# Research-Implementation/AudioVidSum-A-Multi-Modal-Approach-to-Video-Summarization

Hardware: AMD Instinct MI355X
Metric: frames/sec end-to-end (extract+fuse+score), 224x224 + 16kHz (higher is better)
Workload: dtype f16x2; 1 GPU; configs[1]: SumMe-shape batch, 25 videos x ~1800 frames (45143 frames/GPU), visual-only resnet50 extractor (batch-stat BN, the reference's 4-frame BatchNorm micro-batches inside each video) + AVBiLSTM attention scorer + mean-threshold selection; frames_per_gpu=45143, videos_per_gpu=25, extractor=resnet50, frames_per_group=4, chunk_frames=16384, parallelism=videos sharded x1, no data-path collective, selected_frames_rank0=22823

## Files before the change

### audiovidsum-a-multi-modal-approach-to-video-summarization_amd/_abi.py

```python
import ctypes
import os
from ctypes import POINTER, c_char_p, c_double, c_float, c_int, c_int64, c_size_t, c_uint, c_void_p

import torch

_PKG_DIR = os.path.dirname(os.path.abspath(__file__))
STUDY = os.environ.get("AVS_STUDY_LIB") == "1"
_FLAVOUR = os.environ.get("AVS_STUDY_LIB")
LIB_PATH = os.path.join(_PKG_DIR, "lib", "libavsum_hip_study.so" if STUDY else
                        "libavsum_hip_fp16emu.so" if _FLAVOUR == "fp16emu" else "libavsum_hip.so")
HEADER_PATH = os.path.join(os.path.dirname(_PKG_DIR), "include", "avsum_hip.h")

AVS_F32, AVS_BF16, AVS_F32_ACC64, AVS_F32_SPLIT, AVS_F16X2 = 0, 1, 2, 3, 4
AVS_W_ROWS, AVS_W_KSTEP32 = 0, 1
TILE_AUTO, TILE_128, TILE_256, TILE_224, STAGING_GENERIC = 0, 1, 2, 3, 4
CLUSTER_PACKED = 8
X_F16P8, Y_F16P8, RES_F16P8 = 1, 2, 4
LSTM_AUTO, LSTM_STREAM, LSTM_RESIDENT_20_8, LSTM_RESIDENT_16_8 = 0, 1, 2, 3
LSTM_SPLIT4 = 4
ACT_NONE, ACT_RELU = 0, 1
BIAS_NONE, BIAS_COL, BIAS_ROW = 0, 1, 2
E_UNSUPPORTED = -6


class AvsError(RuntimeError):
    pass


class ConvDesc(ctypes.Structure):
    _fields_ = [
        ("dtype", c_int),
        ("n", c_int), ("h", c_int), ("w", c_int),
        ("cin", c_int), ("kh", c_int), ("kw", c_int),
        ("sh", c_int), ("sw", c_int), ("ph", c_int), ("pw", c_int),
        ("ho", c_int), ("wo", c_int), ("cout", c_int),
        ("x_img_stride", c_int64), ("x_row_stride", c_int64), ("x_px_stride", c_int64),
        ("w_row_stride", c_int64), ("y_px_stride", c_int64),
        ("act", c_int), ("alpha", c_float), ("w_layout", c_int), ("variant", c_int), ("formats", c_int),
    ]


P = c_void_p
_SIGNATURES = {
    "avs_abi_version": (c_int, []),
    "avs_last_error": (c_char_p, []),
    "avs_device_info": (c_int, [c_int, POINTER(c_int), POINTER(c_int), POINTER(c_int64), c_char_p, c_int]),
    "avs_f16x2_pack_f32": (c_int, [P, P, c_int64, P]),
    "avs_f16x2_unpack_f32": (c_int, [P, P, c_int64, P]),
    "avs_f16p8_pack_f32": (c_int, [P, P, c_int64, P]),
# ... 158 lines not shown
```

### audiovidsum-a-multi-modal-approach-to-video-summarization_amd/cnn.py

```python
from typing import NamedTuple

import torch
import torch.nn as nn

from . import ops

RESNET_MEAN = (0.485, 0.456, 0.406)
RESNET_STD = (0.229, 0.224, 0.225)


class _NoTorchForward(nn.Module):
    def forward(self, *a, **k):
        raise RuntimeError("this module only holds parameters; the trunk runs through the HIP runner")


class Bottleneck(_NoTorchForward):
    expansion = 4

    def __init__(self, inplanes, planes, stride=1, downsample=None):
        super().__init__()
        self.conv1 = nn.Conv2d(inplanes, planes, 1, bias=False)
        self.bn1 = nn.BatchNorm2d(planes)
        self.conv2 = nn.Conv2d(planes, planes, 3, stride, 1, bias=False)
        self.bn2 = nn.BatchNorm2d(planes)
# ... 50 lines not shown
        self.kstep = ops.weights_kstep32(rows) if rows.shape[1] % step == 0 else None

    def conv_operand(self):
        return (self.kstep, 1) if self.kstep is not None else (self.rows, 0)


class Step(NamedTuple):
    name: str
    form: str
    inp: str = "finished"
    out: str = "finished"
    res: str = "none"
    block: int = -1
    geom: tuple = None
    cluster: int = 1
    packed: bool = False


class ResNet50Runner:

    def __init__(self, trunk, dtype=torch.float32, bn_mode="batch", f32_split=False):
        if bn_mode not in ("batch", "folded"):
            raise ValueError("bn_mode must be 'batch' (reference-faithful) or 'folded'")
        self.trunk, self.dtype, self.bn_mode = trunk, dtype, bn_mode
        self.h2 = f32_split == "f16x2" and dtype == torch.float32
        self.f32_split = bool(f32_split) and not self.h2 and dtype == torch.float32
        self.code = ops.dtype_code(dtype, "f16x2" if self.h2 else self.f32_split)
        self.ecode = self.code if self.h2 else ops.dtype_code(dtype)
        self.fuse_conv_bn = True
        self.fuse_min_rows, self.fuse_ratio_num, self.fuse_ratio_den = 128, 2, 1
        self.bn_local = True
        self.bn_cluster = True
        self.pack_groups = True
        self.fused_stem = True
        self.stem_raw = True
        self.defer_bn_apply = True
        self.defer_res_apply = True
        self.fold_input_bn = True
        self.gram_finish_min_k = 128
        self.p8_blocks = (0, 1, 3, 4, 5) if self.h2 else ()
        self._key = None
        self._w = None
        self._plans = {}

    block_hook = None

    def _blocks(self):
        for li in range(4):
            for b, blk in enumerate(self.trunk[4 + li]):
                yield f"layer{li + 1}.{b}", blk

    def _pair_ok(self):
        b0 = self.trunk[4][0]
        d = b0.downsample
        return d is not None and b0.conv1.weight[0].numel() == d[0].weight[0].numel() and b0.bn1.eps == d[1].eps

    def _prepare(self):
        key = tuple((p.data_ptr(), p._version) for p in self.trunk.parameters()) + (self.dtype,)
        if self._w is not None and key == self._key:
            return self._w
        t, dt = self.trunk, self.dtype
        pack = ops.f16x2_pack if self.h2 else (lambda r: r)

        def bn(m):
            return (m.weight.detach().float().contiguous(), m.bias.detach().float().contiguous(), float(m.eps),
                    m.running_mean.detach().float(), m.running_var.detach().float())
# ... 144 lines not shown
        return group_frames, gsz, bool((sizes == gsz).all())

    def _conv(self, st, w, x, x_aff, groups, residual=None, res_aff=None):
        (geom, xs, _), (wt, (gamma, beta, eps, rmean, rvar)) = st.geom, w[st.name]
        n, cin, kh, ho, wo, cout = geom[0], geom[3], geom[4], geom[10], geom[11], geom[12]
        dev, dt, stem = x.device, self.dtype, st.block < 0
        relu = not st.name.endswith("downsample")
        act = ops.ACT_RELU if relu else ops.ACT_NONE
        grows, gmax = groups[ho * wo]
        wsel, layout = wt.conv_operand()
        y = torch.empty((n, ho, wo, cout), dtype=dt, device=dev)

        def pooled():
            return torch.empty((n, (ho + 2 - 3) // 2 + 1, (wo + 2 - 3) // 2 + 1, cout), dtype=dt, device=dev)

        if st.form == "gram":
            x2d = x.view(-1, cin)
            if self.h2:
                sc, sf = ops.bn_gram_affine_h2(x2d, wt.rows, gmax, gamma, beta, eps, x_aff, store_input=x_aff is not None)
                if st.out == "p8":
                    y = ops.P8.empty((n, ho, wo, cout), dev)
                ops.conv2d_affine(self.code, n, geom[1], geom[2], cin, geom[6], geom[7], ho, wo, cout, x, *xs, wsel,
                                  wsel.stride(0), y, cout, gmax, sc, sf, residual, relu, res_aff, w_layout=layout)
            else:
                ops.conv1x1_gram_bn(x2d, wt.rows, gmax, gamma, beta, eps, y.view(-1, cout), residual, relu, x_aff, res_aff,
                                    finish_input=cin >= self.gram_finish_min_k)
            return y, None

        def conv(**kw):
            return ops.conv2d_raw(self.code, *geom, x, *xs, wsel, wsel.stride(0), y, cout, algo_k=147 if stem else None,
                                  algo_in_elems=x.numel() if stem else None, w_layout=layout, **kw)

        if st.form in ("local", "cluster"):
            conv(act=act, bnlocal=(gmax, gamma, beta, eps, residual), cluster=st.cluster, packed=st.packed)
            return (ops.pool2d(y, "max", 3, 2, 1, pooled(), code=self.ecode) if stem else y), None
        affine = None
        if st.form == "folded":
            conv()
            scale = (gamma / torch.sqrt(rvar + eps)).contiguous()
            affine, grows, gmax = (scale.view(1, -1), (beta - rmean * scale).contiguous().view(1, -1)), None, 0
        else:
            if x_aff is not None:
                if st.form == "stats" and kh == 3:
                    affine = conv(bnstats=(gmax, gamma, beta, eps), x_affine=(x_aff[0], x_aff[1], True))
                if affine is None:
                    xg = groups[geom[1] * geom[2]]
                    ops.bn_apply(x.view(-1, cin), x_aff[0], x_aff[1], xg[0], xg[1], None, ops.ACT_RELU, x.view(-1, cin),
                                 code=self.ecode)
            if st.form == "stats" and affine is None:
                affine = conv(bnstats=(gmax, gamma, beta, eps))
            elif st.form == "split":
                conv()
                affine = ops.bn_batch_stats(y.view(-1, cout), grows, gamma, beta, eps, code=self.ecode)
            if st.out == "deferred":
                return y, affine
        if stem:
            return ops.bn_maxpool(y, affine[0], affine[1], grows, relu, 3, 2, 1, pooled(), code=self.ecode), None
        ops.bn_apply(y.view(-1, cout), affine[0], affine[1], grows, gmax, residual, act, y.view(-1, cout), code=self.ecode)
        return y, None

    def _gram_pair(self, st, w, x, x_aff, gmax):
        wcat, gcat, bcat, eps, c1n = w[st.name]
        block = st.name.split(".conv1+")[0]
        geom, xs, _ = st.geom
        n, h, cin = geom[0], geom[1], geom[3]
        x2d = x.view(-1, cin)
        if self.h2:
# ... 398 lines not shown
```

### audiovidsum-a-multi-modal-approach-to-video-summarization_amd/csrc/igemm.hip

```cpp
#include "avs_internal.h"
#include "igemm_params.h"
#include <type_traits>

__device__ __attribute__((aligned(16))) unsigned int avs_zero16[4];

#ifdef AVS_STUDY
#define AVS_DEBUG_BIT(p, bit) ((p).debug & (bit))
#else
#define AVS_DEBUG_BIT(p, bit) 0
#endif

#define AVS_GLDS16(src, dst)                                                                        \
  __builtin_amdgcn_global_load_lds((const __attribute__((address_space(1))) void*)(src),            \
                                   (__attribute__((address_space(3))) void*)(dst), 16, 0, 0)

__device__ __forceinline__ void avs_split_bf16(const float4& p0, const float4& p1, bf16x8& hi, bf16x8& lo) {
  const float v[8] = {p0.x, p0.y, p0.z, p0.w, p1.x, p1.y, p1.z, p1.w};
  unsigned h[4], l[4];
#pragma unroll
  for (int j = 0; j < 4; ++j) {
    const unsigned short h0 = avs_f32_to_bf16(v[2 * j]), h1 = avs_f32_to_bf16(v[2 * j + 1]);
    const unsigned short l0 = avs_f32_to_bf16(v[2 * j] - avs_bf16_to_f32(h0));
    const unsigned short l1 = avs_f32_to_bf16(v[2 * j + 1] - avs_bf16_to_f32(h1));
    h[j] = (unsigned)h0 | ((unsigned)h1 << 16);
// ... 1561 lines not shown
                         (pl.tall || (long long)p.K * 4 <= g_rowb_threshold_bytes) &&
                         p.KW == 1 && p.K == p.cin && p.K % 32 == 0 && p.K >= 64 &&
                         p.sh == 1 && p.sw == 1 && p.ph == 0 && p.pw == 0 && p.x_row_stride == (long long)p.Wo * p.x_px_stride &&
                         p.x_img_stride == (long long)p.HoWo * p.x_px_stride && p.x_px_stride % 16 == 0 &&
                         256 * p.x_px_stride * 3 + (long long)p.K * 3 < (1ll << 31),
                     AVS_E_UNSUPPORTED,
                     "%s: an AVS_F16P8 input is taken by avs_conv2d_nhwc_bnstats for 1x1 / stride-1 convolutions on dense rows, "
                     "cin a multiple of 32 (>= 64), the input row stride a multiple of 16", who);
  }
  if (p.affine) {
    pl.tall = !(!narrow && (tile_mode == AVS_TILE_128 || (tile_mode == AVS_TILE_AUTO && p.K <= AVS_RULE_AFFINE_128_MAX_K)));
    if (!pl.tall && (long long)p.K * 4 > g_rowb_threshold_bytes) pl.tall = true;
  }
  pl.tile_rows = p.tile_rows ? p.tile_rows : (pl.tall ? 256 : 128);
  pl.tiles_m = ((long long)p.M + pl.tile_rows - 1) / pl.tile_rows;
  AVS_PLAN_REQUIRE(pl.tiles_m * pl.tiles_n < (1ll << 31), AVS_E_SHAPE, "%s: too many tiles", who);
  pl.grid = pl.tiles_m * pl.tiles_n;

  pl.spatial = !(p.ph == 0 && p.pw == 0 && (p.HoWo / p.Wo - 1) * p.sh + (p.K / (p.cin * p.KW)) - 1 < p.H &&
                 (p.Wo - 1) * p.sw + p.KW - 1 < p.W);
  pl.lin_stride = -1;
  if (!pl.spatial && p.KW == 1 && p.K == p.cin && p.sh == 1 && p.sw == 1) {
    if (p.HoWo == 1)
      pl.lin_stride = p.x_img_stride;
    else if (p.x_row_stride == (long long)p.Wo * p.x_px_stride && p.x_img_stride == (long long)p.HoWo * p.x_px_stride)
      pl.lin_stride = p.x_px_stride;
  }
  if (p.tile_rows && dtype == AVS_F16X2) {
    pl.local224 = igemm_h2_local224_ok(p, dtype, pl.lin_stride);
    AVS_PLAN_REQUIRE(pl.local224 || p.cluster <= 1, AVS_E_UNSUPPORTED, "%s: the clustered form runs on the 224-row tile only", who);
    AVS_PLAN_REQUIRE(pl.local224 || tile_mode != AVS_TILE_224, AVS_E_UNSUPPORTED,
                     "%s: AVS_TILE_224 takes AVS_F16X2, groups of 193..224 rows, cout in multiples of 128, cin in multiples of 16", who);
    if (pl.local224) return AVS_OK;
  }

  pl.epi = EPI_ANY;
  if (p.tile_rows)
    pl.epi = EPI_BNLOCAL;
  else if (p.affine)
    pl.epi = EPI_AFFINE;
  else if (p.bias_mode == AVS_BIAS_NONE && p.act == AVS_ACT_NONE && p.alpha == 1.0f)
    pl.epi = stats ? EPI_STATS : EPI_PLAIN;
  else if (brelu)
    pl.epi = EPI_BRELU;
  const bool fast64_only = !(p.variant & AVS_STAGING_GENERIC) && p.cin % (64 / es) == 0 && p.cin % (128 / es) != 0 && p.K / p.cin <= 32;
  const bool short_k = pl.tall || fast64_only || (long long)p.K * es <= g_rowb_threshold_bytes;
  pl.rowb = short_k ? 64 : 128;
  pl.pipe = pl.rowb == 64 && !pl.acc64 && g_pipe3 && p.K * es > 2 * pl.rowb;
  pl.wr = pl.pipe && pl.tall ? 4 : 2;
  pl.fastk = !pl.acc64 && igemm_fastk_ok(p, pl.lin_stride, es, pl.rowb / es, pl.bn);
  if (pl.spatial && pl.pipe && pl.wr == 4 && pl.fastk && (es == 2 || pl.split == 2)) {
    if (pl.epi == EPI_STATS || pl.epi == EPI_BNLOCAL)
      pl.tap9 = igemm_tap9_ok(p, es);
    else if (pl.epi == EPI_BRELU && pl.split == 2)
      pl.tap9 = igemm_taps_ok(p);
  }
  pl.xin = in_affine && pl.tap9 && pl.split == 2 && pl.epi == EPI_STATS;
  pl.ap8 = p.x_p8 && pl.split == 2 && pl.epi == EPI_STATS && !pl.spatial && pl.pipe && pl.fastk;
  return AVS_OK;
}
#undef AVS_PLAN_REQUIRE

#define AVS_LAUNCH_RET(K)                                     \
  do {                                                        \
    hipLaunchKernelGGL(K, grid, dim3(256), 0, stream, p);     \
    return true;                                              \
// ... 140 lines not shown
  return igemm_run(pl, p, stream, who);
}

static int conv_geometry(const avs_conv_desc* d, bool has_bias, IgemmParams& p, const char* who) {
  AVS_REQUIRE(d != nullptr, AVS_E_ARG, "%s: null descriptor", who);
  AVS_REQUIRE(d->n >= 0 && d->h > 0 && d->w > 0 && d->cin > 0 && d->kh > 0 && d->kw > 0 && d->sh > 0 && d->sw > 0 &&
                  d->ph >= 0 && d->pw >= 0 && d->ho > 0 && d->wo > 0 && d->cout > 0,
              AVS_E_SHAPE, "%s: non-positive extent", who);
  AVS_REQUIRE((d->ho - 1) * d->sh - d->ph + d->kh - 1 < d->h + d->ph &&
                  (d->wo - 1) * d->sw - d->pw + d->kw - 1 < d->w + d->pw,
              AVS_E_SHAPE, "%s: output extent %dx%d exceeds what input %dx%d allows", who, d->ho, d->wo, d->h, d->w);
  const long long rows = (long long)d->n * d->ho * d->wo;
  AVS_REQUIRE(rows < (1ll << 31), AVS_E_SHAPE, "%s: %lld output pixels exceed int32", who, rows);
  p.M = (int)rows;
  p.N = d->cout;
  p.K = d->kh * d->kw * d->cin;
  p.HoWo = d->ho * d->wo;
  p.Wo = d->wo;
  p.H = d->h;
  p.W = d->w;
  p.cin = d->cin;
  p.KW = d->kw;
  p.sh = d->sh;
  p.sw = d->sw;
  p.ph = d->ph;
  p.pw = d->pw;
  p.x_img_stride = d->x_img_stride;
  p.x_row_stride = d->x_row_stride;
  p.x_px_stride = d->x_px_stride;
  p.ldb = d->w_row_stride;
  AVS_REQUIRE(d->w_layout == AVS_W_ROWS || d->w_layout == AVS_W_KSTEP32, AVS_E_ARG, "%s: bad w_layout %d", who,
              d->w_layout);
  p.w_kstep = d->w_layout == AVS_W_KSTEP32 ? 1 : 0;
  AVS_REQUIRE((d->variant & ~15) == 0, AVS_E_ARG, "%s: bad variant %d", who, d->variant);
  p.variant = d->variant;
  AVS_REQUIRE((d->formats & ~(AVS_X_F16P8 | AVS_Y_F16P8 | AVS_RES_F16P8)) == 0, AVS_E_ARG, "%s: bad formats %d", who, d->formats);
  AVS_REQUIRE(d->formats == 0 || d->dtype == AVS_F16X2, AVS_E_UNSUPPORTED, "%s: AVS_F16P8 operands belong to the AVS_F16X2 forms", who);
  p.x_p8 = (d->formats & AVS_X_F16P8) ? 1 : 0;
  p.y_p8 = (d->formats & AVS_Y_F16P8) ? 1 : 0;
  p.res_p8 = (d->formats & AVS_RES_F16P8) ? 1 : 0;
  AVS_REQUIRE(!p.w_kstep || (d->dtype != AVS_F32_ACC64 && p.K % (d->dtype == AVS_BF16 ? 32 : 16) == 0), AVS_E_UNSUPPORTED,
              "%s: the reduction-step-major weight layout needs a reduction that is a multiple of a 64-byte step (K = %d)",
              who, p.K);
  p.ldc = d->y_px_stride;
  p.alpha = d->alpha;
  p.act = d->act;
  p.bias_mode = has_bias ? AVS_BIAS_COL : AVS_BIAS_NONE;
  AVS_REQUIRE(p.ldb >= p.K, AVS_E_SHAPE, "%s: w_row_stride %lld < kh*kw*cin=%d", who, p.ldb, p.K);
  return AVS_OK;
}

static void conv_operands(IgemmParams& p, const void* d_x, const void* d_w, const float* d_bias, void* d_y) {
  p.x = (const char*)d_x;
  p.w = (const char*)d_w;
  p.y = (char*)d_y;
  p.bias = d_bias;
}

extern "C" int avs_conv2d_nhwc(const avs_conv_desc* d, const void* d_x, const void* d_w, const float* d_bias,
                               void* d_y, avs_stream_t stream) {
  IgemmParams p{};
  int st = conv_geometry(d, d_bias != nullptr, p, "avs_conv2d_nhwc");
  if (st != AVS_OK) return st;
  conv_operands(p, d_x, d_w, d_bias, d_y);
  return igemm_launch(d->dtype, p, 1, (hipStream_t)stream, "avs_conv2d_nhwc");
}

// ... 132 lines not shown
  AVS_CHECK_LAUNCH(who);
  return AVS_OK;
}

extern "C" int avs_conv2d_nhwc_bnstats(const avs_conv_desc* d, const void* d_x, const void* d_w, void* d_y,
                                       int64_t rows_per_group, const float* d_gamma, const float* d_beta, float eps,
                                       float* d_scale, float* d_shift, void* d_ws, int64_t ws_bytes,
                                       avs_stream_t stream) {
  return conv_bnstats(d, d_x, d_w, d_y, rows_per_group, d_gamma, d_beta, eps, d_scale, d_shift, d_ws, ws_bytes, nullptr,
                      nullptr, 0, stream, "avs_conv2d_nhwc_bnstats");
}

extern "C" int avs_conv2d_nhwc_bnstats_xin(const avs_conv_desc* d, const void* d_x, const void* d_w, void* d_y,
                                           int64_t rows_per_group, const float* d_gamma, const float* d_beta, float eps,
                                           float* d_scale, float* d_shift, void* d_ws, int64_t ws_bytes,
                                           const float* d_in_scale, const float* d_in_shift, int in_relu,
                                           avs_stream_t stream) {
  const char* who = "avs_conv2d_nhwc_bnstats_xin";
  AVS_REQUIRE(d_in_scale && d_in_shift, AVS_E_ARG, "%s: in_scale / in_shift must be given", who);
  return conv_bnstats(d, d_x, d_w, d_y, rows_per_group, d_gamma, d_beta, eps, d_scale, d_shift, d_ws, ws_bytes, d_in_scale,
                      d_in_shift, in_relu, stream, who);
}


static int bnlocal_plan(const avs_conv_desc* d, int64_t rpg, IgemmParams& p, const char* who) {
  int st = conv_geometry(d, false, p, who);
  if (st != AVS_OK) return st;
  AVS_REQUIRE(rpg > 0, AVS_E_ARG, "%s: rows_per_group must be positive", who);
  if (p.M == 0) return AVS_OK;
  const int bn = p.N <= 64 ? 64 : 128;
  const long long per_tile = 256 / rpg;
  const bool h2 = d->dtype == AVS_F16X2;
  const int es = h2 ? 4 : 2;
  const bool ok = (g_bnlocal != 0) && (g_pipe3 != 0) && (d->dtype == AVS_BF16 || h2) && p.N % bn == 0 && p.M % rpg == 0 && rpg <= 256 &&
                  per_tile * rpg * 4 >= 256 * 3 && per_tile <= BNLOCAL_MAX_GROUPS && (long long)p.K * es > 128 &&
                  d->alpha == 1.0f && (p.ldc * es) % (h2 ? 32 : 16) == 0;
  AVS_REQUIRE(ok, AVS_E_UNSUPPORTED,
              "%s: needs bf16 / f16x2, cout a multiple of %d, equal groups of 43..256 rows that fill 3/4 of a 256-row "
              "tile, a reduction of more than 128 bytes, aligned output rows", who, bn);
  p.tiles_n = p.N / bn;
  p.tile_rows = (int)(per_tile * rpg);
  return AVS_OK;
}

static int bncluster_plan(const avs_conv_desc* d, int64_t rpg, int cluster, IgemmParams& p, const char* who) {
  int st = conv_geometry(d, false, p, who);
  if (st != AVS_OK) return st;
  AVS_REQUIRE(rpg > 0 && cluster >= 2 && cluster <= 16, AVS_E_ARG, "%s: rows_per_group > 0 and 2 <= cluster <= 16", who);
  if (p.M == 0) return AVS_OK;
  const bool ok = (g_bnlocal != 0) && (g_pipe3 != 0) && d->dtype == AVS_F16X2 && rpg % cluster == 0 && p.M % rpg == 0 &&
                  rpg / cluster > 192 && rpg / cluster <= 224 && p.N % 128 == 0 && (long long)p.K * 4 > 128 &&
                  d->alpha == 1.0f && (p.ldc * 4) % 32 == 0 && (d->variant & AVS_STAGING_GENERIC) == 0;
  AVS_REQUIRE(ok, AVS_E_UNSUPPORTED,
              "%s: needs AVS_F16X2, equal groups of `cluster` tiles of 193..224 rows each, cout a multiple of 128, a "
              "reduction of more than 128 bytes, aligned output rows", who);
  p.tiles_n = p.N / 128;
  p.tile_rows = (int)(rpg / cluster);
  p.rows_per_group = (int)rpg;
  p.cluster = cluster;
  if (d->variant & AVS_CLUSTER_PACKED) {
    const int64_t per_group = (rpg + 223) / 224;
    AVS_REQUIRE(rpg >= 224 && (rpg % 224 == 0 || rpg % 224 == 112) && per_group <= 16, AVS_E_UNSUPPORTED,
                "%s: AVS_CLUSTER_PACKED needs groups of a multiple of 112 rows, at least 224, that touch at most 16 tiles", who);
    p.tile_rows = 224;
    p.packed = (int)(rpg % 224 ? rpg / 112 : rpg / 224);
  }
  return AVS_OK;
}

static int64_t bncluster_workspace(const IgemmParams& p) {
  if (p.packed) return 64 + (int64_t)((p.M + 223) / 224) * p.tiles_n * 4 * 2 * 64 * 8;
  return 64 + (int64_t)(p.M / p.tile_rows) * p.tiles_n * 4 * 64 * 8;
// ... 149 lines not shown
```

### audiovidsum-a-multi-modal-approach-to-video-summarization_amd/csrc/local224.hip

```cpp
#include "avs_internal.h"
#include "igemm_params.h"
#include <type_traits>
#include <utility>

namespace {
constexpr int L_ROWS = 224;
constexpr int L_MT = L_ROWS / 32;
constexpr int L_BN = 128;
constexpr int L_CPRR = 4;
constexpr int L_STEP = 16;
constexpr int L_BUF = (L_ROWS + L_BN) * L_CPRR;
constexpr int L_P = 32 + 8;
constexpr unsigned L_OOB = 0x80000000u;

template <int OFF>
__device__ __forceinline__ uint4 lds_read_b128_at(unsigned byte_addr) {
  uint4 v;
  asm volatile("ds_read_b128 %0, %1 offset:%2" : "=v"(v) : "v"(byte_addr), "n"(OFF));
  return v;
}
template <int... I>
__device__ __forceinline__ void read_blocks(uint4 (&f)[L_MT], unsigned addr, std::integer_sequence<int, I...>) {
  ((f[I] = lds_read_b128_at<I * 32 * 64>(addr)), ...);
}
}

template <bool SPATIAL>
__global__ __launch_bounds__(256, 2) void igemm_h2_local224_kernel(IgemmParams p) {
  __shared__ uint4 lds[3 * L_BUF];

  const unsigned nwg = gridDim.x, orig = blockIdx.x;
  const unsigned q = nwg >> 3, rr = nwg & 7, xcd = orig & 7;
  const unsigned wg = (xcd < rr ? xcd * (q + 1) : rr * (q + 1) + (xcd - rr) * q) + (orig >> 3);
  int tn = wg % p.tiles_n;
  int tm = wg / p.tiles_n;
  if (p.packed) {
    const unsigned u_t = (unsigned)p.packed, tnn = (unsigned)p.tiles_n;
    const unsigned tiles_m = nwg / tnn;
    const unsigned full = (56u % u_t == 0u) ? (tiles_m / 56u) * 56u : 0u;
    if (orig < full * tnn) {
      const unsigned su = orig / (56u * tnn), l = orig - su * (56u * tnn);
      tn = (int)(l / 56u);
      tm = (int)(su * 56u + l % 56u);
    } else {
      const unsigned o2 = orig - full * tnn, unit = u_t * tnn;
      const unsigned u = o2 / unit, l = o2 - u * unit;
      const unsigned left = tiles_m - full - u * u_t, ul = left < u_t ? left : u_t;
      tn = (int)(l / ul);
      tm = (int)(full + u * u_t + l % ul);
    }
  } else if (p.cluster > 1) {
    const unsigned c = (unsigned)p.cluster, tnn = (unsigned)p.tiles_n;
    const unsigned tiles_m = nwg / tnn;
    const unsigned full = (8u % c == 0u) ? (tiles_m / 8u) * 8u : 0u;
    if (orig < full * tnn) {
      const unsigned su = orig / (8u * tnn), l = orig - su * (8u * tnn);
      tn = (int)(l >> 3);
      tm = (int)(su * 8u + (l & 7u));
    } else {
      const unsigned o2 = orig - full * tnn, unit = c * tnn;
      const unsigned u = o2 / unit, l = o2 - u * unit;
      tn = (int)(l / c);
      tm = (int)(full + u * c + l % c);
    }
  }
  const int m0 = tm * p.tile_rows;
  const int n0 = tn * L_BN;
  const int used = m0 + p.tile_rows <= p.M ? p.tile_rows : p.M - m0;

  const char* __restrict__ x = p.x;
  const char* __restrict__ w = p.w;
  char* __restrict__ y = p.y;

  const int t = threadIdx.x;
  const int wave = __builtin_amdgcn_readfirstlane(t >> 6), lane = t & 63;
  const bool extra = wave < 2;
  const int c = t & (L_CPRR - 1);
  const int rb = t >> 2;
  const int cq = c ^ ((rb >> 2) & (L_CPRR - 1));

  unsigned amask[4], aoff[4], boff[2];
  int f_tap = 0, f_ci0 = 0, f_kw = 0;
  int f_koff = 0;
  int f_kb = 0;
  __amdgpu_buffer_rsrc_t a_rsrc, b_rsrc;
  {
    const int taps = p.K / p.cin;
    long long a_origin;
    int n_first = 0;
    if (p.lin_stride >= 0) {
      a_origin = (long long)m0 * p.lin_stride;
    } else {
      n_first = m0 / p.HoWo;
      a_origin = (long long)n_first * p.x_img_stride - (long long)p.ph * p.x_row_stride - (long long)p.pw * p.x_px_stride;
    }
    a_rsrc = __builtin_amdgcn_make_buffer_rsrc(const_cast<char*>(x) + a_origin * 4, 0, (int)L_OOB, 0x00020000);
    b_rsrc = __builtin_amdgcn_make_buffer_rsrc(
        const_cast<char*>(w) + (p.w_kstep ? (long long)n0 * 64 : (long long)n0 * p.ldb * 4), 0, (int)L_OOB, 0x00020000);
#pragma unroll
    for (int i = 0; i < 4; ++i) {
      unsigned mk = 0, off = L_OOB;
      const int r = rb + 64 * i;
      if (r < used) {
        const int m = m0 + r;
        if (p.lin_stride >= 0) {
          mk = ~0u;
          off = (unsigned)((long long)r * p.lin_stride * 4) + cq * 16;
        } else {
          const int n = m / p.HoWo;
          const int rem = m - n * p.HoWo;
          const int ho = rem / p.Wo;
          const int wo = rem - ho * p.Wo;
          const int hi0 = ho * p.sh - p.ph, wi0 = wo * p.sw - p.pw;
          if constexpr (SPATIAL) {
            for (int tp = 0; tp < taps; ++tp) {
              const int th = tp / p.KW, tw = tp - th * p.KW;
              if ((unsigned)(hi0 + th) < (unsigned)p.H && (unsigned)(wi0 + tw) < (unsigned)p.W) mk |= 1u << tp;
            }
          } else {
            mk = ~0u;
          }
          off = (unsigned)(((long long)(n - n_first) * p.x_img_stride + (long long)(hi0 + p.ph) * p.x_row_stride +
                            (long long)(wi0 + p.pw) * p.x_px_stride) * 4) + cq * 16;
        }
      }
      amask[i] = mk;
      aoff[i] = off;
    }
#pragma unroll
    for (int i = 0; i < 2; ++i)
      boff[i] = p.w_kstep ? (unsigned)((rb + 64 * i) * 64) + (unsigned)(cq >> 2) * (unsigned)p.N * 64u + (cq & 3) * 16
                          : (unsigned)((long long)(rb + 64 * i) * p.ldb * 4) + cq * 16;
  }

  auto stage = [&](int buf) {
    uint4* abuf = lds + buf * L_BUF + wave * 64;
    uint4* bbuf = abuf + L_ROWS * L_CPRR;
#pragma unroll
    for (int i = 0; i < 3; ++i) {
      unsigned off = aoff[i];
      if constexpr (SPATIAL) off = ((amask[i] >> f_tap) & 1u) ? off : L_OOB;
      __builtin_amdgcn_raw_ptr_buffer_load_lds(a_rsrc, (__attribute__((address_space(3))) void*)(abuf + 256 * i), 16,
                                               (int)off, f_koff, 0, 0);
    }
    if (extra) {
      unsigned off = aoff[3];
      if constexpr (SPATIAL) off = ((amask[3] >> f_tap) & 1u) ? off : L_OOB;
      __builtin_amdgcn_raw_ptr_buffer_load_lds(a_rsrc, (__attribute__((address_space(3))) void*)(abuf + 256 * 3), 16,
                                               (int)off, f_koff, 0, 0);
    }
#pragma unroll
    for (int i = 0; i < 2; ++i)
      __builtin_amdgcn_raw_ptr_buffer_load_lds(b_rsrc, (__attribute__((address_space(3))) void*)(bbuf + 256 * i), 16,
                                               (int)boff[i], f_kb, 0, 0);
    f_kb += p.w_kstep ? p.N * 64 : L_STEP * 4;
    f_ci0 += L_STEP;
    f_koff += L_STEP * 4;
    if (f_ci0 == p.cin) {
      f_ci0 = 0;
      ++f_tap;
      f_koff += (int)((p.x_px_stride - p.cin) * 4);
      if (++f_kw == p.KW) {
        f_kw = 0;
        f_koff += (int)((p.x_row_stride - (long long)p.KW * p.x_px_stride) * 4);
      }
    }
  };

  const int lr = lane & 31, lh = lane >> 5;

  f32x16 acc[L_MT];
#pragma unroll
  for (int i = 0; i < L_MT; ++i)
#pragma unroll
    for (int e = 0; e < 16; ++e) acc[i][e] = 0.f;

  const unsigned lds_base = (unsigned)(unsigned long long)((__attribute__((address_space(3))) char*)lds);
  unsigned fa_off[2], fb_off[2];
#pragma unroll
  for (int hl = 0; hl < 2; ++hl) {
    const int chunk = 2 * lh + hl;
    fa_off[hl] = (unsigned)(lr * L_CPRR + (chunk ^ ((lr >> 2) & (L_CPRR - 1)))) * 16u;
    const int brow = wave * 32 + lr;
    fb_off[hl] = (unsigned)((L_ROWS + brow) * L_CPRR + (chunk ^ ((brow >> 2) & (L_CPRR - 1)))) * 16u;
  }

  const int col = n0 + wave * 32 + lr;
  const float inv_n = 1.f / (float)p.tile_rows;
  const int lim = used - 4 * lh;
  const int rl0 = lane >> 2, grp = lane & 3;
  const int col8 = n0 + wave * 32 + grp * 8;
  constexpr int DEPTH = 6;
  uint4 rhi[DEPTH][2], rlo[DEPTH][2];
  auto res_fetch = [&](auto blk) {
    constexpr int mt = decltype(blk)::value;
    const long long row0 = (long long)m0 + mt * 32 + rl0;
    const char* base = p.residual + (row0 * p.ldr + col8) * 4;
#pragma unroll
    for (int it = 0; it < 2; ++it) {
      const bool ok = mt * 32 + rl0 + 16 * it < used;
      const uint4* rp = reinterpret_cast<const uint4*>(ok ? base + (long long)it * 16 * p.ldr * 4 : p.residual);
      rhi[mt % DEPTH][it] = rp[0];
      rlo[mt % DEPTH][it] = rp[1];
    }
  };
  if (p.residual) {
    res_fetch(std::integral_constant<int, 0>{});
    res_fetch(std::integral_constant<int, 1>{});
    res_fetch(std::integral_constant<int, 2>{});
  }

  const int steps = p.K / L_STEP;
  stage(0);
  if (steps > 1) stage(1);
  int cur = 0;
  for (int s = 0; s < steps; ++s) {
    if (s + 1 < steps) {
      if (extra)
        asm volatile("s_waitcnt vmcnt(6)" ::: "memory");
      else
        asm volatile("s_waitcnt vmcnt(5)" ::: "memory");
    } else {
      asm volatile("s_waitcnt vmcnt(0)" ::: "memory");
    }
    __builtin_amdgcn_s_barrier();
    const unsigned bbase = lds_base + (unsigned)cur * (L_BUF * 16u);
    uint4 fah[L_MT], fal[L_MT], fbh, fbl;
    fbh = avs_lds_read_b128(bbase + fb_off[0]);
    read_blocks(fah, bbase + fa_off[0], std::make_integer_sequence<int, L_MT>{});
    fbl = avs_lds_read_b128(bbase + fb_off[1]);
    read_blocks(fal, bbase + fa_off[1], std::make_integer_sequence<int, L_MT>{});
    if (s + 2 < steps) stage(cur == 0 ? 2 : cur - 1);
    asm volatile("s_waitcnt lgkmcnt(%0)" ::"n"(1 + L_MT) : "memory");
    avs_pin(fbh);
#pragma unroll
    for (int mt = 0; mt < L_MT; ++mt) avs_pin(fah[mt]);
    __builtin_amdgcn_sched_barrier(0);
#pragma unroll
    for (int mt = 0; mt < L_MT; ++mt)
      acc[mt] = __builtin_amdgcn_mfma_f32_32x32x16_f16(__builtin_bit_cast(avs_f16x8, fah[mt]),
                                                       __builtin_bit_cast(avs_f16x8, fbh), acc[mt], 0, 0, 0);
    asm volatile("s_waitcnt lgkmcnt(0)" ::: "memory");
    avs_pin(fbl);
#pragma unroll
    for (int mt = 0; mt < L_MT; ++mt) avs_pin(fal[mt]);
    __builtin_amdgcn_sched_barrier(0);
#pragma unroll
    for (int mt = 0; mt < L_MT; ++mt) {
      acc[mt] = __builtin_amdgcn_mfma_f32_32x32x16_f16(__builtin_bit_cast(avs_f16x8, fal[mt]),
                                                       __builtin_bit_cast(avs_f16x8, fbh), acc[mt], 0, 0, 0);
      acc[mt] = __builtin_amdgcn_mfma_f32_32x32x16_f16(__builtin_bit_cast(avs_f16x8, fah[mt]),
                                                       __builtin_bit_cast(avs_f16x8, fbl), acc[mt], 0, 0, 0);
    }
    __builtin_amdgcn_sched_barrier(0);
    cur = cur == 2 ? 0 : cur + 1;
  }

  if (p.residual) {
    res_fetch(std::integral_constant<int, 3>{});
    res_fetch(std::integral_constant<int, 4>{});
    res_fetch(std::integral_constant<int, 5>{});
  }
  const int seg0 = p.packed ? (int)min((long long)used, (m0 / p.rows_per_group + 1ll) * p.rows_per_group - m0) : used;
  const bool shared = seg0 < used;
  float mean, mean_b, s2, s2b = 0.f;
  if (p.packed) {
    float s1 = 0.f, s1b = 0.f;
#pragma unroll
    for (int mt = 0; mt < L_MT; ++mt)
#pragma unroll
      for (int e = 0; e < 16; ++e) {
        if (mt < 3 || (mt == 3 && e < 8))
          s1 += acc[mt][e];
        else
          s1b += acc[mt][e];
      }
    s1 += __shfl_xor(s1, 32, 64);
    s1b += __shfl_xor(s1b, 32, 64);
    const float inv0 = 1.f / (float)seg0, inv1 = 1.f / (float)(shared ? used - seg0 : seg0);
    mean = (shared ? s1 : s1 + s1b) * inv0;
    mean_b = shared ? s1b * inv1 : mean;
    s2 = 0.f;
#pragma unroll
    for (int mt = 0; mt < L_MT; ++mt)
#pragma unroll
      for (int e = 0; e < 16; ++e) {
        const int roff = mt * 32 + (e & 3) + 8 * (e >> 2);
        if (mt < 3 || (mt == 3 && e < 8)) {
// ... 178 lines not shown
      dst[1] = lo;
    }
    asm volatile("s_waitcnt lgkmcnt(0)" ::: "memory");
    __builtin_amdgcn_wave_barrier();
    if constexpr (mt + DEPTH < L_MT) {
      if (p.residual) res_fetch(std::integral_constant<int, mt + DEPTH>{});
    }
  };
  emit(std::integral_constant<int, 0>{});
  emit(std::integral_constant<int, 1>{});
  emit(std::integral_constant<int, 2>{});
  emit(std::integral_constant<int, 3>{});
  emit(std::integral_constant<int, 4>{});
  emit(std::integral_constant<int, 5>{});
  emit(std::integral_constant<int, 6>{});
}

bool igemm_h2_local224_ok(const IgemmParams& p, int dtype, long long lin_stride) {
  const int tile_mode = p.variant & 3;
  if (dtype != AVS_F16X2 || !(tile_mode == AVS_TILE_AUTO || tile_mode == AVS_TILE_224)) return false;
  if (p.variant & AVS_STAGING_GENERIC) return false;
  const int cl = p.cluster > 1 ? p.cluster : 1;
  if (p.packed) {
    if (p.tile_rows != L_ROWS || p.cluster <= 1 || p.rows_per_group < L_ROWS || p.rows_per_group % (L_ROWS / 2) != 0) return false;
  } else if (p.tile_rows * cl != p.rows_per_group || p.tile_rows <= 192 || p.tile_rows > L_ROWS) {
    return false;
  }
  if (p.N % L_BN != 0 || p.M % p.rows_per_group != 0) return false;
  if (p.cin % L_STEP != 0 || p.K % L_STEP != 0 || p.K % p.cin != 0 || p.K / p.cin > 32) return false;
  return igemm_buffer_window_ok(p, lin_stride, 4, L_BN);
}

void igemm_h2_local224_launch(const IgemmParams& p, bool spatial, dim3 grid, hipStream_t stream) {
  if (spatial)
    hipLaunchKernelGGL(igemm_h2_local224_kernel<true>, grid, dim3(256), 0, stream, p);
  else
    hipLaunchKernelGGL(igemm_h2_local224_kernel<false>, grid, dim3(256), 0, stream, p);
}
```

### audiovidsum-a-multi-modal-approach-to-video-summarization_amd/ops.py

```python
import ctypes
from ctypes import c_float, c_void_p

import numpy as np
import torch

from . import _abi
from ._abi import (ACT_NONE, ACT_RELU, AVS_BF16, AVS_F16X2, AVS_F32, AVS_F32_SPLIT, BIAS_COL, BIAS_NONE, BIAS_ROW, check,
                   lib)
from .ragged import (EVAL_CHUNK, EVAL_MAX_T, EVAL_TILE, FUSION_MAX_N, FUSION_MID_L, FUSION_SMALL_L,
                     SHOT_INTERVAL, SHOT_MAX_FRAMES, SHOT_MICRO_BATCH, SUMMARY_MAX_CAPACITY, SUMMARY_MAX_ROWS, EvalTables,
                     FusionTables, RaggedOffsets, SeqTable, ShotTables, SummaryTables)

__all__ = [
    "ACT_NONE", "ACT_RELU", "linear", "gemm_nt_batched", "conv2d", "conv2d_raw", "conv2d_split", "conv_bnlocal_tile_rows", "conv_bncluster_ok", "conv_bnstats_ok", "cluster_exchange_errors", "lstm_split_errors", "conv1x1_bn", "conv1x1_gram_bn", "bn_gram_affine", "gram_supported", "frames_normalize", "pull_copy", "stem_conv_bn_pool", "stem_h2_operands", "stem_conv_pool_h2", "resize_bilinear",
    "bn_batch_stats", "bn_apply", "bn_maxpool", "pool2d", "global_avgpool", "segment_mean", "hsv_frame_diff", "reflect_pad", "stft_f64", "stft_mel_fused", "power_mel",
    "clamp_topdb", "stft_mel_max", "stft_mel_segmean", "stft_mel_segmean_batch", "stft_mel_shots", "vggish_examples", "fill", "quantize", "resample", "lstm", "mha_batchaxis", "score_head", "mhsa_flash", "softmax_rows", "cdist", "dtw_path",
    "gather_scale", "FusionTables", "fusion_batch", "EvalTables", "eval_counts", "segment_mean_mask", "dtype_code", "f16x2_pack", "f16x2_unpack", "bn_gram_affine_h2", "conv2d_affine",
    "SeqTable", "seq_shift_rows", "seq_mse",
    "ShotTables", "hsv_frame_diff_batch", "shot_cuts_batch", "shot_tables", "gather_rows",
    "SummaryTables", "shot_value_sums", "knapsack_batch", "mask_overlap_counts",
]


def _stream():
    return c_void_p(torch.cuda.current_stream().cuda_stream)


class LaunchProfiler:

    def __init__(self, count_only=False, prealloc=0, sample_every=1):
        self.records = []
        self.count_only = count_only
        self.count = 0
        self.sample_every = max(1, int(sample_every))
        self.seen = {}
        self._pool = [(torch.cuda.Event(enable_timing=True), torch.cuda.Event(enable_timing=True))
                      for _ in range(prealloc)]

    def events(self):
        if self._pool:
            return self._pool.pop()
# ... 1573 lines not shown
```

### include/avsum_hip.h

```cpp
#ifndef AVSUM_HIP_H
#define AVSUM_HIP_H

#include <stdint.h>

#ifdef __cplusplus
extern "C" {
#endif

#define AVS_ABI_VERSION 5

enum {
  AVS_OK = 0,
  AVS_E_ARG = -1,
  AVS_E_SHAPE = -2,
  AVS_E_ALIGN = -3,
  AVS_E_HIP = -4,
  AVS_E_WORKSPACE = -5,
  AVS_E_UNSUPPORTED = -6
};

enum { AVS_F32 = 0, AVS_BF16 = 1, AVS_F32_ACC64 = 2, AVS_F32_SPLIT = 3, AVS_F16X2 = 4 };
enum { AVS_ACT_NONE = 0, AVS_ACT_RELU = 1 };
enum { AVS_BIAS_NONE = 0, AVS_BIAS_COL = 1, AVS_BIAS_ROW = 2 };

// ... 1 lines not shown

int avs_abi_version(void);
const char* avs_last_error(void);
int avs_device_info(int dev, int* cu_count, int* clock_khz, int64_t* hbm_bytes,
                    char* arch, int arch_len);

int avs_f16x2_pack_f32(const float* d_src, void* d_dst, int64_t n, avs_stream_t stream);
int avs_f16x2_unpack_f32(const void* d_src, float* d_dst, int64_t n, avs_stream_t stream);

int avs_f16p8_pack_f32(const float* d_src, void* d_dst, int64_t n, avs_stream_t stream);
int avs_f16p8_unpack_f32(const void* d_src, float* d_dst, int64_t n, avs_stream_t stream);


typedef struct {
  int dtype;
  int n, h, w;
  int cin, kh, kw;
  int sh, sw, ph, pw;
  int ho, wo, cout;
  int64_t x_img_stride;
  int64_t x_row_stride;
  int64_t x_px_stride;
  int64_t w_row_stride;
  int64_t y_px_stride;
  int act;
  float alpha;
  int w_layout;
  int variant;
  int formats;
} avs_conv_desc;
enum { AVS_W_ROWS = 0, AVS_W_KSTEP32 = 1 };
enum { AVS_X_F16P8 = 1, AVS_Y_F16P8 = 2, AVS_RES_F16P8 = 4 };
enum { AVS_TILE_AUTO = 0, AVS_TILE_128 = 1, AVS_TILE_256 = 2, AVS_TILE_224 = 3, AVS_STAGING_GENERIC = 4,
       AVS_CLUSTER_PACKED = 8 };

int avs_conv2d_nhwc(const avs_conv_desc* desc, const void* d_x, const void* d_w,
                    const float* d_bias, void* d_y, avs_stream_t stream);
int avs_conv2d_nhwc_split(const avs_conv_desc* desc, const void* d_x, const void* d_w, const float* d_bias, void* d_y,
                          int n_split, void* d_y2, int64_t y2_px_stride, int relu_cols, avs_stream_t stream);

int64_t avs_conv2d_bnstats_workspace_bytes(const avs_conv_desc* desc, int64_t rows_per_group);
int avs_conv2d_nhwc_bnstats(const avs_conv_desc* desc, const void* d_x, const void* d_w, void* d_y,
                            int64_t rows_per_group, const float* d_gamma, const float* d_beta, float eps,
                            float* d_scale, float* d_shift, void* d_ws, int64_t ws_bytes, avs_stream_t stream);
int avs_conv2d_nhwc_bnstats_xin(const avs_conv_desc* desc, const void* d_x, const void* d_w, void* d_y,
                                int64_t rows_per_group, const float* d_gamma, const float* d_beta, float eps,
                                float* d_scale, float* d_shift, void* d_ws, int64_t ws_bytes, const float* d_in_scale,
                                const float* d_in_shift, int in_relu, avs_stream_t stream);

int avs_conv2d_bnlocal_tile_rows(const avs_conv_desc* desc, int64_t rows_per_group);
int avs_conv2d_nhwc_bnlocal(const avs_conv_desc* desc, const void* d_x, const void* d_w, void* d_y,
                            int64_t rows_per_group, const float* d_gamma, const float* d_beta, float eps,
                            const void* d_residual, int64_t ldr, avs_stream_t stream);

int64_t avs_conv2d_bncluster_workspace_bytes(const avs_conv_desc* desc, int64_t rows_per_group, int cluster);
int avs_conv2d_nhwc_bncluster(const avs_conv_desc* desc, const void* d_x, const void* d_w, void* d_y,
                              int64_t rows_per_group, int cluster, const float* d_gamma, const float* d_beta, float eps,
                              const void* d_residual, int64_t ldr, void* d_xchg, int64_t xchg_bytes, uint32_t epoch,
                              avs_stream_t stream);
int avs_bn_gram_affine_f16x2(const void* d_x, int64_t lin_stride, int k, const float* d_in_scale,
                             const float* d_in_shift, const void* d_w, int64_t ldb, int n, int64_t rows_per_group,
                             int groups, const float* d_gamma, const float* d_beta, float eps, float* d_scale,
                             float* d_shift, void* d_a_out, int64_t lda, avs_stream_t stream);
int avs_conv2d_nhwc_affine(const avs_conv_desc* desc, const void* d_x, const void* d_w, void* d_y,
                           int64_t rows_per_group, const float* d_scale, const float* d_shift,
                           const void* d_residual, int64_t ldr, const float* d_res_scale, const float* d_res_shift,
                           avs_stream_t stream);
// ... 266 lines not shown
```

Measured before the change: 27310 frames/s.

## Load 224-row local conv weights straight to registers instead of through LDS

The 224-row f16x2 local-BN conv kernel now fetches its B (weight) fragments with per-lane buffer loads into registers, double-buffered one step ahead, instead of staging them through LDS. LDS then holds only the A tiles, and the old LDS staging path stays selectable through a new AVS_WEIGHTS_LDS variant bit. The change also lets this kernel accept short reductions (K of 128 bytes or less) that were rejected before. The aim is to cut LDS traffic and footprint and widen the set of layers that can use this path. In exchange it adds global/L2 weight traffic per wave, raises register pressure, and changes the vmcnt wait accounting.

```diff
diff --git a/audiovidsum-a-multi-modal-approach-to-video-summarization_amd/_abi.py b/audiovidsum-a-multi-modal-approach-to-video-summarization_amd/_abi.py
--- a/audiovidsum-a-multi-modal-approach-to-video-summarization_amd/_abi.py
+++ b/audiovidsum-a-multi-modal-approach-to-video-summarization_amd/_abi.py
@@ -15,6 +15,7 @@
 AVS_W_ROWS, AVS_W_KSTEP32 = 0, 1
 TILE_AUTO, TILE_128, TILE_256, TILE_224, STAGING_GENERIC = 0, 1, 2, 3, 4
 CLUSTER_PACKED = 8
+WEIGHTS_LDS = 16
 X_F16P8, Y_F16P8, RES_F16P8 = 1, 2, 4
 LSTM_AUTO, LSTM_STREAM, LSTM_RESIDENT_20_8, LSTM_RESIDENT_16_8 = 0, 1, 2, 3
 LSTM_SPLIT4 = 4
diff --git a/audiovidsum-a-multi-modal-approach-to-video-summarization_amd/cnn.py b/audiovidsum-a-multi-modal-approach-to-video-summarization_amd/cnn.py
--- a/audiovidsum-a-multi-modal-approach-to-video-summarization_amd/cnn.py
+++ b/audiovidsum-a-multi-modal-approach-to-video-summarization_amd/cnn.py
@@ -106,6 +106,7 @@
         self.bn_local = True
         self.bn_cluster = True
         self.pack_groups = True
+        self.weights_lds = False
         self.fused_stem = True
         self.stem_raw = True
         self.defer_bn_apply = True
@@ -316,7 +317,8 @@
                                   algo_in_elems=x.numel() if stem else None, w_layout=layout, **kw)
 
         if st.form in ("local", "cluster"):
-            conv(act=act, bnlocal=(gmax, gamma, beta, eps, residual), cluster=st.cluster, packed=st.packed)
+            conv(act=act, bnlocal=(gmax, gamma, beta, eps, residual), cluster=st.cluster, packed=st.packed,
+                 variant=ops.WEIGHTS_LDS if self.weights_lds else 0)
             return (ops.pool2d(y, "max", 3, 2, 1, pooled(), code=self.ecode) if stem else y), None
         affine = None
         if st.form == "folded":
diff --git a/audiovidsum-a-multi-modal-approach-to-video-summarization_amd/csrc/igemm.hip b/audiovidsum-a-multi-modal-approach-to-video-summarization_amd/csrc/igemm.hip
--- a/audiovidsum-a-multi-modal-approach-to-video-summarization_amd/csrc/igemm.hip
+++ b/audiovidsum-a-multi-modal-approach-to-video-summarization_amd/csrc/igemm.hip
@@ -1617,6 +1617,7 @@
     AVS_PLAN_REQUIRE(pl.local224 || tile_mode != AVS_TILE_224, AVS_E_UNSUPPORTED,
                      "%s: AVS_TILE_224 takes AVS_F16X2, groups of 193..224 rows, cout in multiples of 128, cin in multiples of 16", who);
     if (pl.local224) return AVS_OK;
+    AVS_PLAN_REQUIRE((long long)p.K * 4 > 128, AVS_E_UNSUPPORTED, "%s: only the 224-row tile takes a reduction of at most 128 bytes", who);
   }
 
   pl.epi = EPI_ANY;
@@ -1823,7 +1824,7 @@
   AVS_REQUIRE(d->w_layout == AVS_W_ROWS || d->w_layout == AVS_W_KSTEP32, AVS_E_ARG, "%s: bad w_layout %d", who,
               d->w_layout);
   p.w_kstep = d->w_layout == AVS_W_KSTEP32 ? 1 : 0;
-  AVS_REQUIRE((d->variant & ~15) == 0, AVS_E_ARG, "%s: bad variant %d", who, d->variant);
+  AVS_REQUIRE((d->variant & ~31) == 0, AVS_E_ARG, "%s: bad variant %d", who, d->variant);
   p.variant = d->variant;
   AVS_REQUIRE((d->formats & ~(AVS_X_F16P8 | AVS_Y_F16P8 | AVS_RES_F16P8)) == 0, AVS_E_ARG, "%s: bad formats %d", who, d->formats);
   AVS_REQUIRE(d->formats == 0 || d->dtype == AVS_F16X2, AVS_E_UNSUPPORTED, "%s: AVS_F16P8 operands belong to the AVS_F16X2 forms", who);
@@ -2022,12 +2023,16 @@
   const long long per_tile = 256 / rpg;
   const bool h2 = d->dtype == AVS_F16X2;
   const int es = h2 ? 4 : 2;
+  const int tile_mode = d->variant & 3;
+  const bool short_ok = h2 && rpg > 192 && rpg <= 224 && p.N % 128 == 0 && p.K % 16 == 0 && !(d->variant & AVS_STAGING_GENERIC) &&
+                        (tile_mode == AVS_TILE_AUTO || tile_mode == AVS_TILE_224);
   const bool ok = (g_bnlocal != 0) && (g_pipe3 != 0) && (d->dtype == AVS_BF16 || h2) && p.N % bn == 0 && p.M % rpg == 0 && rpg <= 256 &&
-                  per_tile * rpg * 4 >= 256 * 3 && per_tile <= BNLOCAL_MAX_GROUPS && (long long)p.K * es > 128 &&
+                  per_tile * rpg * 4 >= 256 * 3 && per_tile <= BNLOCAL_MAX_GROUPS && ((long long)p.K * es > 128 || short_ok) &&
                   d->alpha == 1.0f && (p.ldc * es) % (h2 ? 32 : 16) == 0;
   AVS_REQUIRE(ok, AVS_E_UNSUPPORTED,
               "%s: needs bf16 / f16x2, cout a multiple of %d, equal groups of 43..256 rows that fill 3/4 of a 256-row "
-              "tile, a reduction of more than 128 bytes, aligned output rows", who, bn);
+              "tile, a reduction of more than 128 bytes (AVS_F16X2 groups of 193..224 rows: of whole 64-byte steps), aligned "
+              "output rows", who, bn);
   p.tiles_n = p.N / bn;
   p.tile_rows = (int)(per_tile * rpg);
   return AVS_OK;
diff --git a/audiovidsum-a-multi-modal-approach-to-video-summarization_amd/csrc/local224.hip b/audiovidsum-a-multi-modal-approach-to-video-summarization_amd/csrc/local224.hip
--- a/audiovidsum-a-multi-modal-approach-to-video-summarization_amd/csrc/local224.hip
+++ b/audiovidsum-a-multi-modal-approach-to-video-summarization_amd/csrc/local224.hip
@@ -9,6 +9,7 @@
 constexpr int L_BN = 128;
 constexpr int L_CPRR = 4;
 constexpr int L_STEP = 16;
+constexpr int L_ABUF = L_ROWS * L_CPRR;
 constexpr int L_BUF = (L_ROWS + L_BN) * L_CPRR;
 constexpr int L_P = 32 + 8;
 constexpr unsigned L_OOB = 0x80000000u;
@@ -25,9 +26,19 @@
 }
 }
 
-template <bool SPATIAL>
+__device__ __forceinline__ void lds224_load_b(uint4& hi, uint4& lo, unsigned voff, u32x4 rsrc, int soff) {
+  asm volatile(
+      "buffer_load_dwordx4 %0, %2, %3, %4 offen\n\t"
+      "buffer_load_dwordx4 %1, %2, %3, %4 offen offset:16"
+      : "=&v"(hi), "=&v"(lo)
+      : "v"(voff), "s"(rsrc), "s"(soff)
+      : "memory");
+}
+
+template <bool SPATIAL, bool BLDS>
 __global__ __launch_bounds__(256, 2) void igemm_h2_local224_kernel(IgemmParams p) {
-  __shared__ uint4 lds[3 * L_BUF];
+  constexpr int BUF = BLDS ? L_BUF : L_ABUF;
+  __shared__ uint4 lds[3 * BUF];
 
   const unsigned nwg = gridDim.x, orig = blockIdx.x;
   const unsigned q = nwg >> 3, rr = nwg & 7, xcd = orig & 7;
@@ -84,6 +95,8 @@
   int f_koff = 0;
   int f_kb = 0;
   __amdgpu_buffer_rsrc_t a_rsrc, b_rsrc;
+  u32x4 w_rsrc;
+  int f_wb = 0;
   {
     const int taps = p.K / p.cin;
     long long a_origin;
@@ -95,8 +108,10 @@
       a_origin = (long long)n_first * p.x_img_stride - (long long)p.ph * p.x_row_stride - (long long)p.pw * p.x_px_stride;
     }
     a_rsrc = __builtin_amdgcn_make_buffer_rsrc(const_cast<char*>(x) + a_origin * 4, 0, (int)L_OOB, 0x00020000);
-    b_rsrc = __builtin_amdgcn_make_buffer_rsrc(
-        const_cast<char*>(w) + (p.w_kstep ? (long long)n0 * 64 : (long long)n0 * p.ldb * 4), 0, (int)L_OOB, 0x00020000);
+    const char* const w0 = w + (p.w_kstep ? (long long)n0 * 64 : (long long)n0 * p.ldb * 4);
+    b_rsrc = __builtin_amdgcn_make_buffer_rsrc(const_cast<char*>(w0), 0, (int)L_OOB, 0x00020000);
+    const unsigned long long wa = (unsigned long long)w0;
+    w_rsrc = u32x4{(unsigned)wa, (unsigned)(wa >> 32) & 0xffffu, L_OOB, 0x00020000u};
 #pragma unroll
     for (int i = 0; i < 4; ++i) {
       unsigned mk = 0, off = L_OOB;
@@ -134,8 +149,7 @@
   }
 
   auto stage = [&](int buf) {
-    uint4* abuf = lds + buf * L_BUF + wave * 64;
-    uint4* bbuf = abuf + L_ROWS * L_CPRR;
+    uint4* abuf = lds + buf * BUF + wave * 64;
 #pragma unroll
     for (int i = 0; i < 3; ++i) {
       unsigned off = aoff[i];
@@ -149,11 +163,14 @@
       __builtin_amdgcn_raw_ptr_buffer_load_lds(a_rsrc, (__attribute__((address_space(3))) void*)(abuf + 256 * 3), 16,
                                                (int)off, f_koff, 0, 0);
     }
-#pragma unroll
-    for (int i = 0; i < 2; ++i)
-      __builtin_amdgcn_raw_ptr_buffer_load_lds(b_rsrc, (__attribute__((address_space(3))) void*)(bbuf + 256 * i), 16,
-                                               (int)boff[i], f_kb, 0, 0);
-    f_kb += p.w_kstep ? p.N * 64 : L_STEP * 4;
+    if constexpr (BLDS) {
+      uint4* bbuf = abuf + L_ROWS * L_CPRR;
+#pragma unroll
+      for (int i = 0; i < 2; ++i)
+        __builtin_amdgcn_raw_ptr_buffer_load_lds(b_rsrc, (__attribute__((address_space(3))) void*)(bbuf + 256 * i), 16,
+                                                 (int)boff[i], f_kb, 0, 0);
+      f_kb += p.w_kstep ? p.N * 64 : L_STEP * 4;
+    }
     f_ci0 += L_STEP;
     f_koff += L_STEP * 4;
     if (f_ci0 == p.cin) {
@@ -167,7 +184,7 @@
     }
   };
 
-  const int lr = lane & 31, lh = lane >> 5;
+  int lr = lane & 31, lh = lane >> 5;
 
   f32x16 acc[L_MT];
 #pragma unroll
@@ -185,11 +202,11 @@
     fb_off[hl] = (unsigned)((L_ROWS + brow) * L_CPRR + (chunk ^ ((brow >> 2) & (L_CPRR - 1)))) * 16u;
   }
 
-  const int col = n0 + wave * 32 + lr;
+  int col = n0 + wave * 32 + lr;
   const float inv_n = 1.f / (float)p.tile_rows;
-  const int lim = used - 4 * lh;
-  const int rl0 = lane >> 2, grp = lane & 3;
-  const int col8 = n0 + wave * 32 + grp * 8;
+  int lim = used - 4 * lh;
+  int rl0 = lane >> 2, grp = lane & 3;
+  int col8 = n0 + wave * 32 + grp * 8;
   constexpr int DEPTH = 6;
   uint4 rhi[DEPTH][2], rlo[DEPTH][2];
   auto res_fetch = [&](auto blk) {
@@ -211,49 +228,85 @@
   }
 
   const int steps = p.K / L_STEP;
-  stage(0);
-  if (steps > 1) stage(1);
+  const unsigned w_off = col >= p.N ? L_OOB
+                         : p.w_kstep ? (unsigned)((wave * 32 + lr) * 64 + 32 * lh)
+                                     : (unsigned)((long long)(wave * 32 + lr) * p.ldb * 4) + 32u * lh;
+  const int w_step = p.w_kstep ? p.N * 64 : L_STEP * 4;
   int cur = 0;
-  for (int s = 0; s < steps; ++s) {
+  auto step = [&](int s, auto next_kind, uint4& bh, uint4& bl, uint4& nh, uint4& nl) {
+    constexpr int NEXT = decltype(next_kind)::value;
     if (s + 1 < steps) {
       if (extra)
-        asm volatile("s_waitcnt vmcnt(6)" ::: "memory");
+        asm volatile("s_waitcnt vmcnt(%0)" ::"n"(BLDS ? 6 : 4) : "memory");
       else
-        asm volatile("s_waitcnt vmcnt(5)" ::: "memory");
+        asm volatile("s_waitcnt vmcnt(%0)" ::"n"(BLDS ? 5 : 3) : "memory");
     } else {
       asm volatile("s_waitcnt vmcnt(0)" ::: "memory");
     }
     __builtin_amdgcn_s_barrier();
-    const unsigned bbase = lds_base + (unsigned)cur * (L_BUF * 16u);
-    uint4 fah[L_MT], fal[L_MT], fbh, fbl;
-    fbh = avs_lds_read_b128(bbase + fb_off[0]);
+    const unsigned bbase = lds_base + (unsigned)cur * (BUF * 16u);
+    uint4 fah[L_MT], fal[L_MT];
+    if constexpr (BLDS) bh = avs_lds_read_b128(bbase + fb_off[0]);
     read_blocks(fah, bbase + fa_off[0], std::make_integer_sequence<int, L_MT>{});
-    fbl = avs_lds_read_b128(bbase + fb_off[1]);
+    if constexpr (BLDS) bl = avs_lds_read_b128(bbase + fb_off[1]);
     read_blocks(fal, bbase + fa_off[1], std::make_integer_sequence<int, L_MT>{});
+    if constexpr (!BLDS && NEXT != 0) {
+      if (NEXT == 1 || s + 1 < steps) {
+        lds224_load_b(nh, nl, w_off, w_rsrc, f_wb);
+        f_wb += w_step;
+      }
+    }
     if (s + 2 < steps) stage(cur == 0 ? 2 : cur - 1);
-    asm volatile("s_waitcnt lgkmcnt(%0)" ::"n"(1 + L_MT) : "memory");
-    avs_pin(fbh);
+    asm volatile("s_waitcnt lgkmcnt(%0)" ::"n"(L_MT + (BLDS ? 1 : 0)) : "memory");
+    avs_pin(bh);
 #pragma unroll
     for (int mt = 0; mt < L_MT; ++mt) avs_pin(fah[mt]);
     __builtin_amdgcn_sched_barrier(0);
 #pragma unroll
     for (int mt = 0; mt < L_MT; ++mt)
       acc[mt] = __builtin_amdgcn_mfma_f32_32x32x16_f16(__builtin_bit_cast(avs_f16x8, fah[mt]),
-                                                       __builtin_bit_cast(avs_f16x8, fbh), acc[mt], 0, 0, 0);
+                                                       __builtin_bit_cast(avs_f16x8, bh), acc[mt], 0, 0, 0);
     asm volatile("s_waitcnt lgkmcnt(0)" ::: "memory");
-    avs_pin(fbl);
+    avs_pin(bl);
 #pragma unroll
     for (int mt = 0; mt < L_MT; ++mt) avs_pin(fal[mt]);
     __builtin_amdgcn_sched_barrier(0);
 #pragma unroll
     for (int mt = 0; mt < L_MT; ++mt) {
       acc[mt] = __builtin_amdgcn_mfma_f32_32x32x16_f16(__builtin_bit_cast(avs_f16x8, fal[mt]),
-                                                       __builtin_bit_cast(avs_f16x8, fbh), acc[mt], 0, 0, 0);
+                                                       __builtin_bit_cast(avs_f16x8, bh), acc[mt], 0, 0, 0);
       acc[mt] = __builtin_amdgcn_mfma_f32_32x32x16_f16(__builtin_bit_cast(avs_f16x8, fah[mt]),
-                                                       __builtin_bit_cast(avs_f16x8, fbl), acc[mt], 0, 0, 0);
+                                                       __builtin_bit_cast(avs_f16x8, bl), acc[mt], 0, 0, 0);
     }
     __builtin_amdgcn_sched_barrier(0);
     cur = cur == 2 ? 0 : cur + 1;
+  };
+  uint4 b0h, b0l, b1h, b1l;
+  if constexpr (BLDS) {
+    stage(0);
+    if (steps > 1) stage(1);
+    for (int s = 0; s < steps; ++s) step(s, std::integral_constant<int, 0>{}, b0h, b0l, b0h, b0l);
+  } else {
+    lds224_load_b(b0h, b0l, w_off, w_rsrc, 0);
+    f_wb = w_step;
+    stage(0);
+    if (steps > 1) stage(1);
+    int s = 0;
+    for (; s + 1 < steps; s += 2) {
+      step(s, std::integral_constant<int, 1>{}, b0h, b0l, b1h, b1l);
+      step(s + 1, std::integral_constant<int, 2>{}, b1h, b1l, b0h, b0l);
+    }
+    if (s < steps) step(s, std::integral_constant<int, 0>{}, b0h, b0l, b1h, b1l);
+  }
+
+  if constexpr (!BLDS) {
+    int lane_e = lane;
+    asm volatile("" : "+v"(lane_e));
+    lr = lane_e & 31, lh = lane_e >> 5;
+    col = n0 + wave * 32 + lr;
+    lim = used - 4 * lh;
+    rl0 = lane_e >> 2, grp = lane_e & 3;
+    col8 = n0 + wave * 32 + grp * 8;
   }
 
   if (p.residual) {
@@ -498,8 +551,16 @@
 }
 
 void igemm_h2_local224_launch(const IgemmParams& p, bool spatial, dim3 grid, hipStream_t stream) {
-  if (spatial)
-    hipLaunchKernelGGL(igemm_h2_local224_kernel<true>, grid, dim3(256), 0, stream, p);
-  else
-    hipLaunchKernelGGL(igemm_h2_local224_kernel<false>, grid, dim3(256), 0, stream, p);
-}
+  const bool blds = (p.variant & AVS_WEIGHTS_LDS) != 0;
+  if (spatial) {
+    if (blds)
+      hipLaunchKernelGGL((igemm_h2_local224_kernel<true, true>), grid, dim3(256), 0, stream, p);
+    else
+      hipLaunchKernelGGL((igemm_h2_local224_kernel<true, false>), grid, dim3(256), 0, stream, p);
+  } else {
+    if (blds)
+      hipLaunchKernelGGL((igemm_h2_local224_kernel<false, true>), grid, dim3(256), 0, stream, p);
+    else
+      hipLaunchKernelGGL((igemm_h2_local224_kernel<false, false>), grid, dim3(256), 0, stream, p);
+  }
+}
diff --git a/audiovidsum-a-multi-modal-approach-to-video-summarization_amd/ops.py b/audiovidsum-a-multi-modal-approach-to-video-summarization_amd/ops.py
--- a/audiovidsum-a-multi-modal-approach-to-video-summarization_amd/ops.py
+++ b/audiovidsum-a-multi-modal-approach-to-video-summarization_amd/ops.py
@@ -5,8 +5,8 @@
 import torch
 
 from . import _abi
-from ._abi import (ACT_NONE, ACT_RELU, AVS_BF16, AVS_F16X2, AVS_F32, AVS_F32_SPLIT, BIAS_COL, BIAS_NONE, BIAS_ROW, check,
-                   lib)
+from ._abi import (ACT_NONE, ACT_RELU, AVS_BF16, AVS_F16X2, AVS_F32, AVS_F32_SPLIT, BIAS_COL, BIAS_NONE, BIAS_ROW,
+                   WEIGHTS_LDS, check, lib)
 from .ragged import (EVAL_CHUNK, EVAL_MAX_T, EVAL_TILE, FUSION_MAX_N, FUSION_MID_L, FUSION_SMALL_L,
                      SHOT_INTERVAL, SHOT_MAX_FRAMES, SHOT_MICRO_BATCH, SUMMARY_MAX_CAPACITY, SUMMARY_MAX_ROWS, EvalTables,
                      FusionTables, RaggedOffsets, SeqTable, ShotTables, SummaryTables)
diff --git a/include/avsum_hip.h b/include/avsum_hip.h
--- a/include/avsum_hip.h
+++ b/include/avsum_hip.h
@@ -57,7 +57,7 @@
 enum { AVS_W_ROWS = 0, AVS_W_KSTEP32 = 1 };
 enum { AVS_X_F16P8 = 1, AVS_Y_F16P8 = 2, AVS_RES_F16P8 = 4 };
 enum { AVS_TILE_AUTO = 0, AVS_TILE_128 = 1, AVS_TILE_256 = 2, AVS_TILE_224 = 3, AVS_STAGING_GENERIC = 4,
-       AVS_CLUSTER_PACKED = 8 };
+       AVS_CLUSTER_PACKED = 8, AVS_WEIGHTS_LDS = 16 };
 
 int avs_conv2d_nhwc(const avs_conv_desc* desc, const void* d_x, const void* d_w,
                     const float* d_bias, void* d_y, avs_stream_t stream);
```

Result: no change. 27390 frames/s, median of 6 (+0.3%).
